# arancormonk/dsd-neo

Measured on AMD Instinct MI355X. Metric: I/Q Msamples/s end-to-end (demod->FEC->MBE) per GPU; % HBM roofline, higher is better.
Workload: dtype f32

## Files before the change

### dsd-neo_amd/csrc/ddn_rx.hip

```cpp

#include <hip/hip_runtime.h>
#include <cstdio>
#include <cstdlib>
#include <mutex>
#include <stdint.h>

#include "ddn_device.h"
#include "ddn_p25h_dev.h"
#include "ddn_slicer_dev.h"
#include "ddn_tables_p25.h"

using ddn_sl::two_max_insert;
using ddn_sl::two_min_insert;

#define DDN_RXW_RAW (1 << 30)
namespace {
constexpr int TS = 64;
constexpr int SS = 128;
constexpr int MS = 1024;
constexpr int NT = DDN_P25_FILTER_TAPS;
constexpr int QCAP = 10;
constexpr uint32_t kSyncBits = 0xFB30A0u;

__constant__ uint32_t c_taps[NT];
// ... 573 lines not shown
v_max2(float a, float b) {
    float r;
    asm("v_max_f32 %0, %1, %2" : "=v"(r) : "v"(a), "v"(b));
    return r;
}
__device__ __forceinline__ float
v_min3(float a, float b, float c) {
    float r;
    asm("v_min3_f32 %0, %1, %2, %3" : "=v"(r) : "v"(a), "v"(b), "v"(c));
    return r;
}
__device__ __forceinline__ float
v_max3(float a, float b, float c) {
    float r;
    asm("v_max3_f32 %0, %1, %2, %3" : "=v"(r) : "v"(a), "v"(b), "v"(c));
    return r;
}
__device__ __forceinline__ float
v_med3(float a, float b, float c) {
    float r;
    asm("v_med3_f32 %0, %1, %2, %3" : "=v"(r) : "v"(a), "v"(b), "v"(c));
    return r;
}
__device__ __forceinline__ void
helper_idle(float& spin, bool sleep_instead, int sleep_arg) {
    if (sleep_instead) {
        if (sleep_arg >= 4) {
            __builtin_amdgcn_s_sleep(4);
        } else {
            __builtin_amdgcn_s_sleep(1);
        }
        return;
    }
#pragma unroll
    for (int k = 0; k < 12; k++) {
        asm volatile("v_max_f32 %0, %0, %0" : "+v"(spin));
    }
}
__device__ __forceinline__ float
div5_exact(float x) {
    const float y = 0.2f;
    const float q = x * y;
    const float r = __builtin_fmaf(-5.0f, q, x);
    return __builtin_fmaf(r, y, q);
}


#ifndef DDN_RX_CYCLES
#define DDN_RX_CYCLES 0
#endif

template <int CPW, bool SMALL = false>
struct LdsW {
    static constexpr int TW = CPW <= 8 ? 128 : 64, RTW = 3 * TW;
    static constexpr int WMW = TW == 128 ? (SMALL ? 40 : 64) : (SMALL ? 24 : 32);
    static constexpr int QTW = TW == 128 ? 40 : 20;
    float sb[SS][CPW];
    float lb[24][CPW];
    float sh[24][CPW];
    float raw[CPW][RTW + TW + 13];
    float flt[CPW][RTW + TW + 13];
    alignas(16) float q[2][QTW][CPW][4];
    int qn[2][4];
    int qo[2][CPW];
    alignas(16) float sfx[2][WMW][CPW][4];
    int sidx0[2][CPW];
};

template <int CPW>
struct LdsH {
    float hh[ddn_p25h::HN][CPW][3];
    int req_seq[CPW], req_kind[CPW], req_hw[CPW], req_n[CPW], req_o[CPW], req_neg[CPW], req_nc[CPW];
    int rsp_seq[CPW], rsp_ext[CPW], rsp_more[CPW];
#if DDN_RX_CYCLES
    int req_t[CPW], rsp_t[CPW], rsp_pick[CPW];
#endif
    int tile_done[4];
    int hwid[8];
    int ready[4];
    int fready[4];
    int staged[4];
    float hh_dummy[CPW][4];
    ddn_p25h::Scratch sc;
};

template <int CPW, bool HM, int NRW_T = (HM ? 2 : 1)>
__global__ __launch_bounds__(HM ? 64 * (NRW_T + 2) * (NRW_T == 4 ? 2 : 1) : 192) __attribute__((amdgpu_waves_per_eu(NRW_T == 4 ? 3 : 2))) void
k_p25_rxw(const float* __restrict__ raw, const float* __restrict__ filt, const float* __restrict__ prev_tail,
          float* __restrict__ fstale, long n,
          size_t stride, int n_channels, DdnRxConfig cfg, DdnRxState* __restrict__ state, float* __restrict__ sbuf_store,
          float* __restrict__ lbuf_store, float* __restrict__ shist_store, float* __restrict__ minring,
          float* __restrict__ maxring, uint8_t* __restrict__ rec, uint8_t* __restrict__ flags,
          int32_t* __restrict__ counts, size_t max_sym, const int32_t* __restrict__ lock_cfg,
          DdnP25HState* __restrict__ hstate, float* __restrict__ hh_store, int32_t* __restrict__ events,
          int32_t* __restrict__ n_events) {
    using LW = LdsW<CPW, HM>;
    constexpr int TW = LW::TW, RTW = LW::RTW, WMW = LW::WMW, QTW = LW::QTW;
    (void)RTW;
    extern __shared__ unsigned char smem_all[];
    constexpr int LTHREADS = HM ? 64 * (NRW_T + 2) : 192;
    constexpr size_t LBYTES = HM ? ((((sizeof(LW) + 15) & ~(size_t)15) + sizeof(LdsH<CPW>) + 15) & ~(size_t)15) : sizeof(LW);
    const int lhalf = (NRW_T == 4) ? (int)(threadIdx.x / LTHREADS) : 0;
    const int ltid = (int)threadIdx.x - lhalf * LTHREADS;
    const int lblock = (NRW_T == 4) ? (int)blockIdx.x * 2 + lhalf : (int)blockIdx.x;
    unsigned char* smem_raw = smem_all + (size_t)lhalf * LBYTES;
    LW& L = *reinterpret_cast<LW*>(smem_raw);
    LdsH<CPW>& H = *reinterpret_cast<LdsH<CPW>*>(smem_raw + ((sizeof(LW) + 15) & ~(size_t)15));
    const int lane = ltid & 63;
    const bool fuse_mf = HM && LdsW<CPW, HM>::TW == 128 && cfg.use_filter != 0 && filt == nullptr;
    int wave_role = ltid >> 6;
    if (HM && !(cfg.dbg & 524288)) {
        unsigned hwid;
        asm volatile("s_getreg_b32 %0, hwreg(HW_REG_HW_ID)" : "=s"(hwid));
        if (lane == 0) {
            H.hwid[ltid >> 6] = (int)hwid;
        }
        __syncthreads();
        int seen = 0, slot_of_simd0 = 0;
        for (int w = 0; w < 4; w++) {
            const int v = H.hwid[w];
            seen |= 1 << ((v >> 4) & 3);
            if (((v >> 4) & 3) == 0) {
                slot_of_simd0 = v & 15;
            }
        }
        if (NRW_T == 2 && seen == 15) {
            wave_role = ((int)((hwid >> 4) & 3) - 2 * (slot_of_simd0 & 1)) & 3;
        }
        if (NRW_T == 4) {
            constexpr int NW = NRW_T + 2;
            const int me = ltid >> 6, my_simd = (int)((hwid >> 4) & 3);
            int cnt[4] = {0, 0, 0, 0}, my_rank = 0;
            for (int w = 0; w < NW; w++) {
                const int sd = (H.hwid[w] >> 4) & 3;
                cnt[sd]++;
                my_rank += (w < me && sd == my_simd) ? 1 : 0;
            }
            const bool good = cnt[0] >= 1 && cnt[1] >= 1 && cnt[2] >= 1 && cnt[3] >= 1 && cnt[0] <= 2 && cnt[1] <= 2 && cnt[2] <= 2 && cnt[3] <= 2;
            if (good) {
                int before = 0;
                for (int sd = 0; sd < my_simd; sd++) {
                    before += my_rank == 0 ? 1 : (cnt[sd] == 2 ? 1 : 0);
                }
                wave_role = my_rank == 0 ? before : NRW_T + before;
            }
        }
    }
    const bool hwave = HM && wave_role == NRW_T + 1;
    if (HM && hwave) {
        const int ch0 = lblock * CPW;
        const int ch = ch0 + lane;
        auto wg_barrier = [&]() {
            __builtin_amdgcn_fence(__ATOMIC_RELEASE, "workgroup");
            __builtin_amdgcn_s_barrier();
            __builtin_amdgcn_fence(__ATOMIC_ACQUIRE, "workgroup");
        };
        __builtin_amdgcn_s_setprio(3);
    DdnP25HState hs = DdnP25HState{};
    int h_served = 0, h_nev = 0;
    const bool hlive = hwave && lane < CPW && ch < n_channels;
    {
        if (hlive) {
            hs = hstate[ch];
        }
        for (int k = lane; k < ddn_p25h::HN * CPW * 3; k += 64) {
            const int w = k % 3, c = (k / 3) % CPW, slot = k / (3 * CPW);
            H.hh[slot][c][w] = (ch0 + c < n_channels) ? hh_store[((size_t)(ch0 + c) * ddn_p25h::HN + slot) * 3 + w] : 0.0f;
        }
        if (lane < CPW) {
            H.req_seq[lane] = 0;
            H.rsp_seq[lane] = 0;
        }
        ddn_p25h::crc_cols_fill(H.sc.crc_cols, lane);
        if (lane == 0) {
            for (int w = 0; w < 4; w++) {
                H.tile_done[w] = DDN_RXW_RAW;
                H.ready[w] = 1;
                H.fready[w] = 0;
                H.staged[w] = 1;
            }
            ddn_nid::gf_fill(H.sc.ex, H.sc.lg);
            ddn_nid::chase_masks_fill(H.sc.masks);
        }
    }
        wg_barrier();
        wg_barrier();
    int dbg_pend = 0, dbg_free = 0;
    auto serve = [&](int c, int seq) {
        using namespace ddn_p25h;
        Scratch& sc = H.sc;
        const int kind = H.req_kind[c], hw = H.req_hw[c], nsym = H.req_n[c], o_dec = H.req_o[c], neg = H.req_neg[c];
        const int gch = ch0 + c;
        const long long dbg_t0 = (cfg.dbg & 65536) ? (long long)clock64() : 0;
#if DDN_RX_CYCLES
        if (lane == c) {
            const int since_req = (int)dbg_t0 - H.req_t[c];
            const int since_free = dbg_free == 0 ? 0x7fffffff : (int)((unsigned)(int)dbg_t0 - (unsigned)dbg_free);
            H.rsp_pick[c] = (cfg.dbg & 268435456) ? 1000 * dbg_pend : ((cfg.dbg & 536870912) ? (since_req < since_free ? since_req : since_free) : since_req);
        }
#endif
        int dbg_path = 0;
        long long dbg_s[3] = {0, 0, 0};
        auto dbg_stamp = [&](int k) {
            if (cfg.dbg & 131072) {
                dbg_s[k] = (long long)clock64() - dbg_t0;
            }
        };
        int phase = __shfl(hs.phase, c), block = __shfl(hs.block, c), end = __shfl(hs.end, c), sk0 = __shfl(hs.skipdibit, c);
        int nac = __shfl(hs.nac, c), p2cc = __shfl(hs.p2_cc, c);
        int nev = __shfl(h_nev, c);
        if (H.req_nc[c]) {
            nac = 0;
        }
        if (kind == 1) {
            phase = PH_NID;
        }
        int ext = 0, more = 0;
        int ev_kind = 0, ev_a = 0, ev_b = 0;
        int32_t pay0 = 0, pay1 = 0, pay2 = 0, pay3 = 0;
        auto slice_at = [&](int i, int& d, int& relb, int& l0, int& l1) {
            int slot = hw - nsym + i;
            slot += slot < 0 ? HN : 0;
            const float* e = &H.hh[slot][c][0];
            const float mx = e[1], mn = e[2];
            const float center = (mx + mn) / 2.0f;
            const ddn_sl::Thr th = {center, ((mx - center) * 5.0f / 8.0f) + center, ((mn - center) * 5.0f / 8.0f) + center, mx, mn};
            ddn_sl::slice_soft(e[0], th, neg, d, relb, l0, l1);
        };
        if (phase == PH_NID) {
            bool nid_done = false;
            ddn_nid::NidRes r = {0, 0, 0, 0};
            {
                int hd = 0;
                if (lane < 33 && lane != 11) {
                    int slot = hw - nsym + lane;
                    slot += slot < 0 ? HN : 0;
                    const float* e = &H.hh[slot][c][0];
                    const float mx = e[1], mn = e[2], x = e[0];
                    const float center = (mx + mn) / 2.0f;
                    const float umid = ((mx - center) * 5.0f / 8.0f) + center, lmid = ((mn - center) * 5.0f / 8.0f) + center;
                    hd = (x > center) ? ((x > umid) ? (neg ? 3 : 1) : (neg ? 2 : 0)) : ((x < lmid) ? (neg ? 1 : 3) : (neg ? 0 : 2));
                }
                const unsigned long long bh = __ballot(hd & 2), bl = __ballot(hd & 1);
                const uint32_t ph = (uint32_t)((bh & 0x7FFull) | ((bh >> 12) << 11)), pl = (uint32_t)((bl & 0x7FFull) | ((bl >> 12) << 11));
                auto spread = [](uint32_t v) {
                    uint64_t x = v;
                    x = (x | (x << 16)) & 0x0000FFFF0000FFFFull;
                    x = (x | (x << 8)) & 0x00FF00FF00FF00FFull;
                    x = (x | (x << 4)) & 0x0F0F0F0F0F0F0F0Full;
                    x = (x | (x << 2)) & 0x3333333333333333ull;
                    x = (x | (x << 1)) & 0x5555555555555555ull;
                    return x;
                };
                const uint64_t both = spread(ph) | (spread(pl) << 1);
                const uint64_t w0 = both & 0x7FFFFFFFFFFFFFFFull;
                const int par0 = (int)(both >> 63);
                dbg_stamp(0);
                if (ddn_nid::bch_63_16_is_codeword(w0)) {
                    r = ddn_nid::nid_fields(w0, 0, par0);
                    nid_done = r.status > 0;
                }
                dbg_stamp(2);
// ... 93 lines not shown
                ev_a = block;
                ev_b = crc_ok | (((by[0] >> 8) & 0xFF) << 8) | (((last << 8) | sel) << 16);
                block++;
                if (last || block >= 3) {
                    phase = PH_IDLE;
                } else {
                    ext = 101;
                    more = 1;
                }
            } else {
                if (crc_ok) {
                    const int sap = (by[0] >> 8) & 0x3F, blks = (by[1] >> 16) & 0x7F;
                    end = blks + 1;
                    if ((sap == 61 || sap == 63) && blks > 10) {
                        end = 4;
                    }
                }
                ev_kind = EV_MPDU;
                ev_a = crc_ok;
                ev_b = (end & 0xFFFF) | (byte0 << 16);
                block = 1;
                int total = 0;
                for (int bi = 1; bi < end; bi++) {
                    int ska;
                    total += mpdu_block_symbols(sk0, ska);
                    sk0 = ska;
                }
                ext = total;
                more = 0;
                phase = PH_IDLE;
            }
        } else {
            phase = PH_IDLE;
        }
        if (lane == c) {
            hs.phase = phase;
            hs.block = block;
            hs.end = end;
            hs.skipdibit = sk0;
            hs.nac = nac;
            hs.p2_cc = p2cc;
            h_served = seq;
            H.rsp_ext[c] = ext;
            H.rsp_more[c] = more;
#if DDN_RX_CYCLES
            H.rsp_t[c] = (int)clock64();
#endif
        }
#if DDN_RX_CYCLES
        dbg_free = (int)clock64();
#endif
        if (lane == c) {
            __builtin_amdgcn_fence(__ATOMIC_RELEASE, "workgroup", "local");
            __hip_atomic_store(&H.rsp_seq[c], seq, __ATOMIC_RELAXED, __HIP_MEMORY_SCOPE_WORKGROUP);
            if (ev_kind) {
                if (nev < cfg.max_events && gch < n_channels) {
                    int32_t* e = events + ((size_t)gch * cfg.max_events + nev) * 4;
                    e[0] = o_dec;
                    e[1] = ev_kind;
                    e[2] = ev_a;
                    e[3] = ev_b;
                    if (cfg.event_data) {
                        *reinterpret_cast<int4*>(cfg.event_data + ((size_t)gch * cfg.max_events + nev) * 4) = make_int4(pay0, pay1, pay2, pay3);
                    }
                    if (cfg.dbg & 65536) {
                        e[2] = dbg_path;
                        e[3] = (int)((long long)clock64() - dbg_t0);
                        if (cfg.dbg & 131072) {
                            e[2] = dbg_path | ((int)(dbg_s[0] >> 4) << 4);
                            e[3] = (int)(dbg_s[1] >> 4) | ((int)(dbg_s[2] >> 4) << 16);
                        }
#if DDN_RX_CYCLES
                        if (cfg.dbg & 1073741824) {
                            e[2] = H.rsp_pick[c];
                        }
#endif
                    }
                }
                h_nev = nev + 1;
            }
        }
    };

        constexpr int LPR_H = CPW / NRW_T;
        constexpr int NPASS = LPR_H / 2;
        static_assert(LPR_H % 2 == 0, "the filter pass takes the channels of a recurrence wave in pairs");
        typedef float mf2h __attribute__((ext_vector_type(2)));
        auto mf_pass = [&](int h, int t, int p) {
            const int slot = t % 3;
            const int cA = h * LPR_H + 2 * p, cB = cA + 1;
            const float* ra = &L.raw[cA][TW + slot * TW + 2 * lane - (NT - 1)];
            const float* rb = &L.raw[cB][TW + slot * TW + 2 * lane - (NT - 1)];
            mf2h accA = {0.0f, 0.0f}, accB = {0.0f, 0.0f};
            {
                constexpr int G = 7;
                static_assert(NT == 13 * G, "thirteen groups of seven taps");
                uint32_t la = (uint32_t)(uintptr_t)(const __attribute__((address_space(3))) float*)ra;
                uint32_t lb = (uint32_t)(uintptr_t)(const __attribute__((address_space(3))) float*)rb;
#define DDN_MF_LOAD(d, e, a, b)                                                                                                    \
    asm volatile("ds_read2_b32 %0, %14 offset1:1\n\tds_read2_b32 %7, %15 offset1:1\n\t"                                          \
                 "ds_read2_b32 %1, %14 offset0:1 offset1:2\n\tds_read2_b32 %8, %15 offset0:1 offset1:2\n\t"                     \
                 "ds_read2_b32 %2, %14 offset0:2 offset1:3\n\tds_read2_b32 %9, %15 offset0:2 offset1:3\n\t"                     \
                 "ds_read2_b32 %3, %14 offset0:3 offset1:4\n\tds_read2_b32 %10, %15 offset0:3 offset1:4\n\t"                    \
                 "ds_read2_b32 %4, %14 offset0:4 offset1:5\n\tds_read2_b32 %11, %15 offset0:4 offset1:5\n\t"                    \
                 "ds_read2_b32 %5, %14 offset0:5 offset1:6\n\tds_read2_b32 %12, %15 offset0:5 offset1:6\n\t"                    \
                 "ds_read2_b32 %6, %14 offset0:6 offset1:7\n\tds_read2_b32 %13, %15 offset0:6 offset1:7"                        \
                 : "=&v"(d[0]), "=&v"(d[1]), "=&v"(d[2]), "=&v"(d[3]), "=&v"(d[4]), "=&v"(d[5]), "=&v"(d[6]), "=&v"(e[0]),         \
                   "=&v"(e[1]), "=&v"(e[2]), "=&v"(e[3]), "=&v"(e[4]), "=&v"(e[5]), "=&v"(e[6])                                    \
                 : "v"(a), "v"(b)                                                                                                  \
                 : "memory")
#define DDN_MF_WAIT(d, e, cnt)                                                                                                     \
    asm volatile("s_waitcnt lgkmcnt(" cnt ")"                                                                                      \
                 : "+v"(d[0]), "+v"(d[1]), "+v"(d[2]), "+v"(d[3]), "+v"(d[4]), "+v"(d[5]), "+v"(d[6]), "+v"(e[0]), "+v"(e[1]),     \
                   "+v"(e[2]), "+v"(e[3]), "+v"(e[4]), "+v"(e[5]), "+v"(e[6]))
                mf2h xa0[G], xb0[G], xa1[G], xb1[G];
                DDN_MF_LOAD(xa0, xb0, la, lb);
#pragma unroll
                for (int g = 0; g < 13; g++) {
                    mf2h* ca = (g & 1) ? xa1 : xa0;
                    mf2h* cb = (g & 1) ? xb1 : xb0;
                    if (g + 1 < 13) {
                        la += 4u * G;
                        lb += 4u * G;
                        if (g & 1) {
                            DDN_MF_LOAD(xa0, xb0, la, lb);
                        } else {
                            DDN_MF_LOAD(xa1, xb1, la, lb);
                        }
                        DDN_MF_WAIT(ca, cb, "14");
                    } else {
                        DDN_MF_WAIT(ca, cb, "0");
                    }
#pragma unroll
                    for (int k = 0; k < G; k++) {
                        const float tp = __uint_as_float(ddn_p25_filter_bits[g * G + k]);
                        const mf2h tt = {tp, tp};
                        const mf2h pa = tt * ca[k], pb = tt * cb[k];
                        accA += pa;
                        accB += pb;
                    }
                }
#undef DDN_MF_LOAD
#undef DDN_MF_WAIT
            }
            float* fa = &L.flt[cA][TW + slot * TW + 2 * lane];
            float* fb = &L.flt[cB][TW + slot * TW + 2 * lane];
            fa[0] = accA.x;
            fa[1] = accA.y;
            fb[0] = accB.x;
            fb[1] = accB.y;
            if (slot == 2) {
                fa[-3 * TW] = accA.x;
                fa[1 - 3 * TW] = accA.y;
                fb[-3 * TW] = accB.x;
                fb[1 - 3 * TW] = accB.y;
            }
        };
        const int n_tiles = (int)((n + TW - 1) / TW);
        int mfj[NRW_T], mfp[NRW_T];
        for (int w = 0; w < NRW_T; w++) {
            mfj[w] = 0;
            mfp[w] = 0;
        }
        float idle_spin = 0.0f;
#if DDN_RX_CYCLES
        long long dbg_mf[8] = {0, 0, 0, 0, 0, 0, 0, 0};
#endif
        while (true) {
            const int rq = (lane < CPW) ? __hip_atomic_load(&H.req_seq[lane], __ATOMIC_RELAXED, __HIP_MEMORY_SCOPE_WORKGROUP) : 0;
            const unsigned long long pend = __ballot(lane < CPW && rq != h_served);
            if (pend != 0) {
                __builtin_amdgcn_fence(__ATOMIC_ACQUIRE, "workgroup");
                const int c = __ffsll((long long)pend) - 1;
                dbg_pend = __popcll(pend);
#if DDN_RX_CYCLES
                const long long sv_t0 = (long long)clock64();
#endif
                serve(c, __shfl(rq, c));
#if DDN_RX_CYCLES
                dbg_mf[2] += (long long)clock64() - sv_t0;
                dbg_mf[3]++;
#endif
                continue;
            }
            bool did = false;
            if (fuse_mf) {
                int hsel = -1, jsel = 0x7fffffff;
#pragma unroll
                for (int h = 0; h < NRW_T; h++) {
                    if (mfj[h] < n_tiles && mfj[h] < jsel
                        && __hip_atomic_load(&H.staged[h], __ATOMIC_RELAXED, __HIP_MEMORY_SCOPE_WORKGROUP) > mfj[h]) {
                        hsel = h;
                        jsel = mfj[h];
                    }
                }
                if (hsel >= 0) {
                    __builtin_amdgcn_fence(__ATOMIC_ACQUIRE, "workgroup");
                    int pj = 0;
#pragma unroll
                    for (int h = 0; h < NRW_T; h++) {
                        pj = h == hsel ? mfp[h] : pj;
                    }
#if DDN_RX_CYCLES
                    const long long mf_t0 = (long long)clock64();
#endif
                    mf_pass(hsel, jsel, pj);
#if DDN_RX_CYCLES
                    dbg_mf[0] += (long long)clock64() - mf_t0;
                    dbg_mf[1]++;
#endif
                    pj++;
                    const bool tile_filtered = pj == NPASS;
#pragma unroll
                    for (int h = 0; h < NRW_T; h++) {
                        if (h == hsel) {
                            mfp[h] = tile_filtered ? 0 : pj;
                            mfj[h] += tile_filtered ? 1 : 0;
                        }
                    }
                    if (tile_filtered) {
                        __builtin_amdgcn_fence(__ATOMIC_RELEASE, "workgroup");
                        if (lane == 0) {
                            __hip_atomic_store(&H.fready[hsel], jsel + 1, __ATOMIC_RELAXED, __HIP_MEMORY_SCOPE_WORKGROUP);
                        }
                    }
                    did = true;
                }
            }
            if (did) {
                continue;
            }
            bool all_done = true;
            for (int w = 0; w < NRW_T; w++) {
                all_done = all_done
                           && (__hip_atomic_load(&H.tile_done[w], __ATOMIC_ACQUIRE, __HIP_MEMORY_SCOPE_WORKGROUP) & (DDN_RXW_RAW - 1)) >= n_tiles;
            }
            if (all_done) {
                break;
            }
            helper_idle(idle_spin, (cfg.dbg & 8388608) != 0, 4);
#if DDN_RX_CYCLES
            dbg_mf[4]++;
#endif
        }
#if DDN_RX_CYCLES
        if ((cfg.dbg & 8192) && lane == 0) {
            uint8_t* d = rec + ((size_t)ch0 + 1) * max_sym * 10 - 448;
            for (int k = 0; k < 64; k++) {
                d[k] = reinterpret_cast<const uint8_t*>(dbg_mf)[k];
            }
        }
#endif
    {
        if (hlive) {
            hstate[ch] = hs;
            n_events[ch] = h_nev;
        }
        for (int k = lane; k < ddn_p25h::HN * CPW * 3; k += 64) {
            const int w = k % 3, c = (k / 3) % CPW, slot = k / (3 * CPW);
            if (ch0 + c < n_channels) {
                hh_store[((size_t)(ch0 + c) * ddn_p25h::HN + slot) * 3 + w] = H.hh[slot][c][w];
            }
        }
    }
        return;
    }
    constexpr int NRW = NRW_T;
    constexpr int LPR = CPW / NRW;
    const int wave = wave_role;
    const bool loader = wave == NRW;
    const bool winprep = wave == (HM ? NRW : NRW + 1);
    const bool recur = wave < NRW;
    const int rw = recur ? wave : 0;
    const int ch0 = lblock * CPW;
    const int ln = rw * LPR + (lane < LPR ? lane : 0);
    const int ch = ch0 + ln;
    const bool live = recur && lane < LPR && ch < n_channels;
    const bool use_flt = cfg.use_filter != 0;
    const bool ld_flt = use_flt && filt != nullptr;
    const bool raw_always = !ld_flt || (cfg.dbg & 16384) != 0;
    const float inf = __builtin_inff();
    if (recur && !(cfg.dbg & 32768)) {
        __builtin_amdgcn_s_setprio(3);
    }

    DdnRxState s;
    if (live) {
        s = state[ch];
        for (int k = 0; k < SS; k++) {
            L.sb[k][ln] = sbuf_store[(size_t)k * n_channels + ch];
        }
        for (int k = 0; k < 24; k++) {
            L.lb[k][ln] = lbuf_store[(size_t)k * n_channels + ch];
            L.sh[k][ln] = shist_store[(size_t)k * n_channels + ch];
        }
    } else {
        s = DdnRxState{};
    }
    float wabs = 0.0f;
    if (live) {
        L.sidx0[0][ln] = s.sidx;
        for (int k = 0; k < SS; k++) {
            wabs = fmaxf(wabs, fabsf(L.sb[k][ln]));
        }
    }
    auto stage = [&](long t0, int slot) {
        const int tn = (int)((n - t0) < TW ? (n - t0) : TW);
        constexpr int RPP = CPW < 16 ? CPW : 16;
#pragma unroll
        for (int half = 0; half < TW / 64; half++) {
// ... 621 lines not shown
        int job[NRW];
        for (int h = 0; h < NRW; h++) {
            job[h] = 0;
        }
        float idle_spin = 0.0f;
        auto jobs_left = [&]() {
            bool any = false;
            for (int h = 0; h < NRW; h++) {
                any = any || job[h] <= n_tiles;
            }
            return any;
        };
        while (jobs_left()) {
            bool served = false;
#pragma unroll
            for (int h = 0; h < NRW; h++) {
                const int j = job[h];
                const int tdw = __hip_atomic_load(&H.tile_done[h], __ATOMIC_RELAXED, __HIP_MEMORY_SCOPE_WORKGROUP);
                if (j > n_tiles || (tdw & (DDN_RXW_RAW - 1)) < j) {
                    continue;
                }
                __builtin_amdgcn_fence(__ATOMIC_ACQUIRE, "workgroup");
                const long long w0 = (DDN_RX_CYCLES && (cfg.dbg & 8192)) ? (long long)clock64() : 0;
                if (j < n_tiles) {
                    long long c0 = w0;
                    StageRegs sg;
                    if (j + 1 < n_tiles) {
                        stage_half_load((long)(j + 1) * TW, h, sg, (tdw & DDN_RXW_RAW) != 0);
                    }
                    if (DDN_RX_CYCLES && (cfg.dbg & 8192)) {
                        const long long c1 = (long long)clock64();
                        dbg_cyc[0] += c1 - c0;
                        c0 = c1;
                    }
                    if (offload && j > 0 && !(cfg.dbg & 512)) {
                        drain_half((j - 1) & 1, h);
                    }
                    if (DDN_RX_CYCLES && (cfg.dbg & 8192)) {
                        const long long c1 = (long long)clock64();
                        dbg_cyc[1] += c1 - c0;
                        c0 = c1;
                    }
                    if (fuse_mf) {
                        if (j + 1 < n_tiles) {
                            stage_half_store(j + 1, h, sg);
                        }
                        __builtin_amdgcn_fence(__ATOMIC_RELEASE, "workgroup");
                        if (lane == 0) {
                            __hip_atomic_store(&H.staged[h], j + 2, __ATOMIC_RELAXED, __HIP_MEMORY_SCOPE_WORKGROUP);
                        }
                        if (DDN_RX_CYCLES && (cfg.dbg & 8192)) {
                            const long long c1 = (long long)clock64();
                            dbg_cyc[0] += c1 - c0;
                            c0 = c1;
                        }
                    }
                    if (j >= 1 && !(cfg.dbg & 256)) {
                        compute_sfx_half(j & 1, j & 1, h);
                    }
                    if (DDN_RX_CYCLES && (cfg.dbg & 8192)) {
                        const long long c1 = (long long)clock64();
                        dbg_cyc[2] += c1 - c0;
                        c0 = c1;
                    }
                    if (!fuse_mf && j + 1 < n_tiles) {
                        stage_half_store(j + 1, h, sg);
                    }
                    if (DDN_RX_CYCLES && (cfg.dbg & 8192)) {
                        dbg_cyc[0] += (long long)clock64() - c0;
                    }
                    __builtin_amdgcn_fence(__ATOMIC_RELEASE, "workgroup");
                    if (lane == 0) {
                        __hip_atomic_store(&H.ready[h], j + 2, __ATOMIC_RELAXED, __HIP_MEMORY_SCOPE_WORKGROUP);
                    }
                } else if (offload && n_tiles > 0) {
                    drain_half((n_tiles - 1) & 1, h);
                }
                if (DDN_RX_CYCLES && (cfg.dbg & 8192)) {
                    dbg_busy += (long long)clock64() - w0;
                }
                job[h] = j + 1;
                served = true;
            }
            if (!served) {
                const long long w0 = (DDN_RX_CYCLES && (cfg.dbg & 8192)) ? (long long)clock64() : 0;
                helper_idle(idle_spin, (cfg.dbg & 8388608) != 0, 1);
                if (DDN_RX_CYCLES && (cfg.dbg & 8192)) {
                    dbg_wait += (long long)clock64() - w0;
                }
            }
        }
        it = n_tiles;
    } else
    for (t0 = 0; t0 < n; t0 += TW, it++) {
        const long long dbg_t0 = (DDN_RX_CYCLES && (cfg.dbg & 8192)) ? (long long)clock64() : 0;
        const int tn = (int)((n - t0) < TW ? (n - t0) : TW);
        const bool more = (t0 + TW) < n;
        long long dbg_spin = 0;
        if (HM) {
            const long long w0 = (DDN_RX_CYCLES && (cfg.dbg & 8192)) ? (long long)clock64() : 0;
            while (__hip_atomic_load(&H.ready[rw], __ATOMIC_RELAXED, __HIP_MEMORY_SCOPE_WORKGROUP) <= it
                   || (fuse_mf && __hip_atomic_load(&H.fready[rw], __ATOMIC_RELAXED, __HIP_MEMORY_SCOPE_WORKGROUP) <= it)) {
                __builtin_amdgcn_s_sleep(1);
            }
            __builtin_amdgcn_fence(__ATOMIC_ACQUIRE, "workgroup");
            if (DDN_RX_CYCLES && (cfg.dbg & 8192)) {
                dbg_spin = (long long)clock64() - w0;
            }
        }
        if (loader || winprep) {
            if (loader) {
                if (more) {
                    stage(t0 + TW, (it + 1) % 3);
                }
                if (offload && it > 0 && !(cfg.dbg & 512)) {
                    drain((it - 1) & 1);
                }
            }
            if (winprep) {
                if (it >= 1 && !(cfg.dbg & 256)) {
                    compute_sfx(it & 1, it & 1);
                }
            }
        } else {
            const int base = TW + (it % 3) * TW;
            auto rd = [&](const float* row, int j) { return row[base + j]; };
            auto cold_limit = [&]() {
                if (!s.filter_on) {
                    return -2147483647;
                }
                const long long d = (long long)(NT - 1) - (abs0 + t0 - s.filt_start);
                return d <= -2147483647LL ? -2147483647 : (d > 1000000LL ? 1000000 : (int)d);
            };
            cold_until = cold_limit();
            if (it >= 1) {
                pp1 = pc1, pp2 = pc2, pp3 = pc3, pp4 = pc4;
                npp = npc;
                sbuf_sel = (it - 1) & 1;
            }
            pc1 = inf, pc2 = inf, pc3 = -inf, pc4 = -inf;
            npc = 0;
            tk = 0;
            itq = it & 1;
            o_tile = o;
            if (live && offload) {
                L.qo[it & 1][ln] = o;
            }
            int guard = 0;
            bool gblocked = false;
            bool respin = false;
            int blk_o = -1;
            while (true) {
                const long long dbg_p0 = (DDN_RX_CYCLES && (cfg.dbg & 8192)) ? (long long)clock64() : 0;
                long long dbg_p1 = 0;
                if (HM && __any(hwait)) {
                    if (hwait
                        && __hip_atomic_load(&H.rsp_seq[ln], __ATOMIC_RELAXED, __HIP_MEMORY_SCOPE_WORKGROUP) == hseq) {
                        __builtin_amdgcn_fence(__ATOMIC_ACQUIRE, "workgroup", "local");
                        const int ext = H.rsp_ext[ln];
                        hwait = false;
                        if ((cfg.dbg & 65536) && !(cfg.dbg & (67108864 | 134217728))) {
                            s.dbg_wait += (long long)clock64();
                        }
#if DDN_RX_CYCLES
                        if (cfg.dbg & 67108864) {
                            s.dbg_wait += (long long)((int)clock64() - H.rsp_t[ln]);
                        }
                        if (cfg.dbg & 134217728) {
                            s.dbg_wait += (long long)H.rsp_pick[ln];
                        }
#endif
                        if (ext > 0) {
                            s.lock_left = ext;
                            s.hn = ext;
                            s.hphase = H.rsp_more[ln] ? 2 : 0;
                        } else {
                            s.hphase = 0;
                            frame_end();
                        }
                    }
                    if (__any(hwait) && (LPR > 4) != ((cfg.dbg & 262144) != 0)) {
                        __builtin_amdgcn_s_sleep(1);
                        continue;
                    }
                }
// ... 992 lines not shown
                    s.in_symbol = 0;
                    commit_pre(sym);
                    int fl = 0;
                    float q_max = 0.0f, q_min = 0.0f;
                    if (s.have_sync) {
                        commit_inframe(sym, done_snap, fl, q_max, q_min);
                    } else {
                        commit_hunt(sym, done_snap, fl);
                    }
                    emit(sym, fl, q_max, q_min);
                }
                gblocked = gblocked || blocked;
            }
            if ((DDN_RX_CYCLES && (cfg.dbg & 8192)) && dbg_kind >= 0) {
                dbg_cyc[dbg_kind] += (long long)clock64() - dbg_prev;
                dbg_n[dbg_kind]++;
                dbg_kind = -1;
            }
            if (offload && lane == 0) {
                L.qn[it & 1][rw] = (tk - 1) < QTW ? (tk - 1) : QTW;
            }
            if (live) {
                L.sidx0[(it + 1) & 1][ln] = s.sidx;
                sp -= TW;
            }
            if (HM) {
                const bool want = live
                                  && (!s.filter_on || cold_until > 0 || (!s.have_sync && s.hunt_pos + 64 >= 1800) || raw_always);
                const int raw_bit = __any(want) ? DDN_RXW_RAW : 0;
                __builtin_amdgcn_fence(__ATOMIC_RELEASE, "workgroup");
                if (lane == 0) {
                    __hip_atomic_store(&H.tile_done[rw], (it + 1) | raw_bit, __ATOMIC_RELAXED, __HIP_MEMORY_SCOPE_WORKGROUP);
                }
            }
        }
        if (DDN_RX_CYCLES && (cfg.dbg & 8192)) {
            const long long t1 = (long long)clock64();
            if (!HM) {
                __syncthreads();
            }
            dbg_busy += t1 - dbg_t0 - dbg_spin;
            dbg_wait += (long long)clock64() - t1 + dbg_spin;
        } else if (!HM) {
            __syncthreads();
        }
    }
    if ((DDN_RX_CYCLES && (cfg.dbg & 8192)) && lane == 0) {
        uint8_t* d = rec + ((size_t)ch0 + 1) * max_sym * 10 - 192 + (wave < NRW ? (wave ? 1 : 0) : 2) * 64;
        const long long v[8] = {dbg_busy, dbg_wait, dbg_cyc[0], dbg_cyc[1], dbg_cyc[2], dbg_n[0], dbg_n[1], dbg_n[2]};
        for (int k = 0; k < 64; k++) {
            d[k] = reinterpret_cast<const uint8_t*>(v)[k];
        }
        if (wave == 0) {
            uint8_t* d2 = rec + ((size_t)ch0 + 1) * max_sym * 10 - 256;
            for (int k = 0; k < 64; k++) {
                d2[k] = reinterpret_cast<const uint8_t*>(dbg_sec)[k];
                d2[k - 64] = reinterpret_cast<const uint8_t*>(dbg_run)[k];
                d2[k - 128] = reinterpret_cast<const uint8_t*>(dbg_blk)[k];
                d2[k - 256] = reinterpret_cast<const uint8_t*>(dbg_ent)[k];
            }
        }
    }
    if (!HM && loader && offload && it > 0) {
        drain((it - 1) & 1);
    }
    if (live) {
        if (s.have_sync) {
            s.umid = ((s.max - s.center) * 5.0f / 8.0f) + s.center;
            s.lmid = ((s.min - s.center) * 5.0f / 8.0f) + s.center;
        }
        s.n_abs = abs0 + n;
        state[ch] = s;
        counts[ch] = o;
        for (int k = 0; k < SS; k++) {
            sbuf_store[(size_t)k * n_channels + ch] = L.sb[k][ln];
        }
        for (int k = 0; k < 24; k++) {
            lbuf_store[(size_t)k * n_channels + ch] = L.lb[k][ln];
            shist_store[(size_t)k * n_channels + ch] = L.sh[k][ln];
        }
    }
}

template <int CPW, bool HM, int NRW_T = (HM ? 2 : 1)>
static hipError_t
launch_rxw(const float* raw, const float* filt, const float* prev_tail, float* fstale, long n, size_t stride, int n_channels,
           const DdnRxConfig& cfg, DdnRxState* state, float* sbuf_store, float* lbuf_store, float* shist_store,
           float* minring, float* maxring, uint8_t* rec, uint8_t* flags, int32_t* counts, size_t max_sym, const int32_t* lock_cfg,
           DdnP25HState* hstate, float* hh_store, int32_t* events, int32_t* n_events, hipStream_t st) {
    const size_t shm1 = HM ? (((((sizeof(LdsW<CPW, true>) + 15) & ~(size_t)15) + sizeof(LdsH<CPW>)) + 15) & ~(size_t)15) : sizeof(LdsW<CPW>);
    const size_t shm = shm1 * (NRW_T == 4 ? 2 : 1);
    const unsigned lblocks = (unsigned)((n_channels + CPW - 1) / CPW);
    const unsigned nblocks = NRW_T == 4 ? (lblocks + 1) / 2 : lblocks;
    const unsigned nthreads = HM ? 64 * (NRW_T + 2) * (NRW_T == 4 ? 2 : 1) : 192;
    if (HM && (cfg.sym_rate <= 0 || cfg.out_rate / cfg.sym_rate < 9)) {
        return hipErrorInvalidValue;
    }
    hipError_t e = hipFuncSetAttribute(reinterpret_cast<const void*>(&k_p25_rxw<CPW, HM, NRW_T>),
                                       hipFuncAttributeMaxDynamicSharedMemorySize, (int)shm);
    if (e != hipSuccess) {
        return e;
    }
    if (DDN_EXP_ENV("DDN_RX_OCC")) {
        int nb = -1;
        hipFuncAttributes fa;
        (void)hipOccupancyMaxActiveBlocksPerMultiprocessor(&nb, reinterpret_cast<const void*>(&k_p25_rxw<CPW, HM, NRW_T>), (int)nthreads, shm);
        (void)hipFuncGetAttributes(&fa, reinterpret_cast<const void*>(&k_p25_rxw<CPW, HM, NRW_T>));
        fprintf(stderr, "k_p25_rxw<%d,%d,%d>: %d blocks per CU, %d regs, %zu B dynamic LDS, %zu B static\n", CPW, (int)HM, NRW_T, nb, fa.numRegs, shm, fa.sharedSizeBytes);
    }
    hipLaunchKernelGGL((k_p25_rxw<CPW, HM, NRW_T>), dim3(nblocks), dim3(nthreads), shm, st, raw,
                       filt, prev_tail, fstale, n, stride, n_channels, cfg, state, sbuf_store, lbuf_store, shist_store, minring,
                       maxring, rec, flags, counts, max_sym, lock_cfg, hstate, hh_store, events, n_events);
    return hipGetLastError();
}

template <int CPW>
static hipError_t
launch_rx(const float* raw, const float* filt, const float* prev_tail, float* fstale, long n, size_t stride, int n_channels,
          const DdnRxConfig& cfg, DdnRxState* state, float* sbuf_store, float* lbuf_store, float* shist_store,
          float* minring, float* maxring, uint8_t* rec, uint8_t* flags, int32_t* counts, size_t max_sym, const int32_t* lock_cfg,
          hipStream_t st) {
    const size_t shm = sizeof(Lds<CPW>);
    hipError_t e = hipFuncSetAttribute(reinterpret_cast<const void*>(&k_p25_rx<CPW>),
                                       hipFuncAttributeMaxDynamicSharedMemorySize, (int)shm);
    if (e != hipSuccess) {
        return e;
    }
    hipLaunchKernelGGL(k_p25_rx<CPW>, dim3((unsigned)((n_channels + CPW - 1) / CPW)), dim3(128), shm, st, raw, filt,
                       prev_tail, fstale, n, stride, n_channels, cfg, state, sbuf_store, lbuf_store, shist_store, minring,
                       maxring, rec, flags, counts, max_sym, lock_cfg);
    return hipGetLastError();
}

static inline bool
use_filter_row_missing(const DdnRxConfig* cfg, const float* filt) {
    return cfg->use_filter && !filt;
}

static int
handler_mode_cpw(int channels_per_wave, int n_channels) {
    int cpw = channels_per_wave;
    if (const char* e = DDN_EXP_ENV("DDN_RX_CPW")) {
        cpw = atoi(e);
    }
    if (cpw != 4 && cpw != 8 && cpw != 16) {
        cpw = n_channels <= 4 * 512 ? 4 : 8;
    }
    return cpw;
}

extern "C" int
ddn_dev_p25_rx_fuses_filter(const DdnRxConfig* cfg, int channels_per_wave, int n_channels) {
    return cfg && cfg->handlers && cfg->use_filter && handler_mode_cpw(channels_per_wave, n_channels) <= 8
               ? 1
               : 0;
}

extern "C" hipError_t
ddn_dev_p25_rx(const float* raw, const float* filt, const float* prev_tail, float* fstale, long n, size_t stride, int n_channels,
               const DdnRxConfig* cfg, DdnRxState* state, float* sbuf_store, float* lbuf_store, float* shist_store,
               float* minring, float* maxring, uint8_t* rec, uint8_t* flags, int32_t* counts, size_t max_sym,
               int channels_per_wave, const int32_t* lock_cfg, DdnP25HState* hstate, float* hh_store, int32_t* events,
               int32_t* n_events, hipStream_t st) {
    if (n_channels <= 0 || n <= 0) {
        return hipSuccess;
    }
    if ((unsigned long long)n_channels * (unsigned long long)MS * 4ull > 0xFFFFFFFFull) {
        return hipErrorInvalidValue;
    }
    {
        static std::mutex mu;
        static bool taps_up[64] = {};
        int dev = 0;
        hipError_t e = hipGetDevice(&dev);
        if (e != hipSuccess) {
            return e;
        }
        std::lock_guard<std::mutex> lock(mu);
        if (dev < 0 || dev >= 64 || !taps_up[dev]) {
            e = hipMemcpyToSymbol(HIP_SYMBOL(c_taps), ddn_p25_filter_bits, sizeof(uint32_t) * NT);
            if (e != hipSuccess) {
                return e;
            }
            if (dev >= 0 && dev < 64) {
                taps_up[dev] = true;
            }
        }
    }
    int cpw = channels_per_wave;
    if (const char* e = DDN_EXP_ENV("DDN_RX_CPW")) {
        cpw = atoi(e);
    }
    const int whole = cfg->sym_rate > 0 ? cfg->out_rate / cfg->sym_rate : 0;
// ... 70 lines not shown
```

Baseline: 25570.

## Share fused matched-filter passes between handler and stager waves via atomic work queue

The fused matched-filter work moves out of per-wave private counters into a shared LDS queue. Both the handler wave and idle stager waves claim filter passes with compare-and-swap and mark completion per pass. A new FUSE template parameter makes the fused path a compile-time instantiation, so non-fused kernels drop the dead code. The aim is to spread the filter load over idle waves so recurrence waves wait less, at the cost of atomic contention and a noinline call in the stager loop.

```diff
diff --git a/dsd-neo_amd/csrc/ddn_rx.hip b/dsd-neo_amd/csrc/ddn_rx.hip
--- a/dsd-neo_amd/csrc/ddn_rx.hip
+++ b/dsd-neo_amd/csrc/ddn_rx.hip
@@ -679,9 +679,134 @@
     int staged[4];
     float hh_dummy[CPW][4];
     ddn_p25h::Scratch sc;
+    int mf_next[4];
+    int mf_done[4][8];
 };
 
-template <int CPW, bool HM, int NRW_T = (HM ? 2 : 1)>
+typedef float mf2h __attribute__((ext_vector_type(2)));
+template <int CPW, int NRW_T>
+__device__ __forceinline__ void
+rxw_mf_pass(LdsW<CPW, true>& L, int lane, int h, int t, int p) {
+    constexpr int TW = LdsW<CPW, true>::TW;
+    constexpr int LPR_H = CPW / NRW_T;
+    static_assert(LPR_H % 2 == 0, "the filter pass takes the channels of a recurrence wave in pairs");
+    const int slot = t % 3;
+    const int cA = h * LPR_H + 2 * p, cB = cA + 1;
+    const float* ra = &L.raw[cA][TW + slot * TW + 2 * lane - (NT - 1)];
+    const float* rb = &L.raw[cB][TW + slot * TW + 2 * lane - (NT - 1)];
+    mf2h accA = {0.0f, 0.0f}, accB = {0.0f, 0.0f};
+    {
+        constexpr int G = 7;
+        static_assert(NT == 13 * G, "thirteen groups of seven taps");
+        uint32_t la = (uint32_t)(uintptr_t)(const __attribute__((address_space(3))) float*)ra;
+        uint32_t lb = (uint32_t)(uintptr_t)(const __attribute__((address_space(3))) float*)rb;
+#define DDN_MF_LOAD(d, e, a, b)                                                                                                    \
+    asm volatile("ds_read2_b32 %0, %14 offset1:1\n\tds_read2_b32 %7, %15 offset1:1\n\t"                                          \
+                 "ds_read2_b32 %1, %14 offset0:1 offset1:2\n\tds_read2_b32 %8, %15 offset0:1 offset1:2\n\t"                     \
+                 "ds_read2_b32 %2, %14 offset0:2 offset1:3\n\tds_read2_b32 %9, %15 offset0:2 offset1:3\n\t"                     \
+                 "ds_read2_b32 %3, %14 offset0:3 offset1:4\n\tds_read2_b32 %10, %15 offset0:3 offset1:4\n\t"                    \
+                 "ds_read2_b32 %4, %14 offset0:4 offset1:5\n\tds_read2_b32 %11, %15 offset0:4 offset1:5\n\t"                    \
+                 "ds_read2_b32 %5, %14 offset0:5 offset1:6\n\tds_read2_b32 %12, %15 offset0:5 offset1:6\n\t"                    \
+                 "ds_read2_b32 %6, %14 offset0:6 offset1:7\n\tds_read2_b32 %13, %15 offset0:6 offset1:7"                        \
+                 : "=&v"(d[0]), "=&v"(d[1]), "=&v"(d[2]), "=&v"(d[3]), "=&v"(d[4]), "=&v"(d[5]), "=&v"(d[6]), "=&v"(e[0]),         \
+                   "=&v"(e[1]), "=&v"(e[2]), "=&v"(e[3]), "=&v"(e[4]), "=&v"(e[5]), "=&v"(e[6])                                    \
+                 : "v"(a), "v"(b)                                                                                                  \
+                 : "memory")
+#define DDN_MF_WAIT(d, e, cnt)                                                                                                     \
+    asm volatile("s_waitcnt lgkmcnt(" cnt ")"                                                                                      \
+                 : "+v"(d[0]), "+v"(d[1]), "+v"(d[2]), "+v"(d[3]), "+v"(d[4]), "+v"(d[5]), "+v"(d[6]), "+v"(e[0]), "+v"(e[1]),     \
+                   "+v"(e[2]), "+v"(e[3]), "+v"(e[4]), "+v"(e[5]), "+v"(e[6]))
+        mf2h xa0[G], xb0[G], xa1[G], xb1[G];
+        DDN_MF_LOAD(xa0, xb0, la, lb);
+#pragma unroll
+        for (int g = 0; g < 13; g++) {
+            mf2h* ca = (g & 1) ? xa1 : xa0;
+            mf2h* cb = (g & 1) ? xb1 : xb0;
+            if (g + 1 < 13) {
+                la += 4u * G;
+                lb += 4u * G;
+                if (g & 1) {
+                    DDN_MF_LOAD(xa0, xb0, la, lb);
+                } else {
+                    DDN_MF_LOAD(xa1, xb1, la, lb);
+                }
+                DDN_MF_WAIT(ca, cb, "14");
+            } else {
+                DDN_MF_WAIT(ca, cb, "0");
+            }
+#pragma unroll
+            for (int k = 0; k < G; k++) {
+                const float tp = __uint_as_float(ddn_p25_filter_bits[g * G + k]);
+                const mf2h tt = {tp, tp};
+                const mf2h pa = tt * ca[k], pb = tt * cb[k];
+                accA += pa;
+                accB += pb;
+            }
+        }
+#undef DDN_MF_LOAD
+#undef DDN_MF_WAIT
+    }
+    float* fa = &L.flt[cA][TW + slot * TW + 2 * lane];
+    float* fb = &L.flt[cB][TW + slot * TW + 2 * lane];
+    fa[0] = accA.x;
+    fa[1] = accA.y;
+    fb[0] = accB.x;
+    fb[1] = accB.y;
+    if (slot == 2) {
+        fa[-3 * TW] = accA.x;
+        fa[1 - 3 * TW] = accA.y;
+        fb[-3 * TW] = accB.x;
+        fb[1 - 3 * TW] = accB.y;
+    }
+}
+
+template <int CPW, int NRW_T>
+__device__ __forceinline__ int
+rxw_mf_take(LdsW<CPW, true>& L, LdsH<CPW>& H, int lane, int mf_tiles) {
+    constexpr int NPASS = CPW / NRW_T / 2;
+    static_assert(LdsW<CPW, true>::TW != 128 || 4 * NPASS <= 8, "H.mf_done holds four tiles' pass words");
+    int hsel = -1, jsel = 0x7fffffff, vsel = 0;
+#pragma unroll
+    for (int h = 0; h < NRW_T; h++) {
+        const int v = __builtin_amdgcn_readfirstlane(__hip_atomic_load(&H.mf_next[h], __ATOMIC_RELAXED, __HIP_MEMORY_SCOPE_WORKGROUP));
+        const int j = v / NPASS;
+        if (j < mf_tiles && j < jsel
+            && __builtin_amdgcn_readfirstlane(__hip_atomic_load(&H.staged[h], __ATOMIC_RELAXED, __HIP_MEMORY_SCOPE_WORKGROUP)) > j) {
+            hsel = h;
+            jsel = j;
+            vsel = v;
+        }
+    }
+    if (hsel < 0) {
+        return 0;
+    }
+    int won = 0;
+    if (lane == 0) {
+        int expect = vsel;
+        won = __hip_atomic_compare_exchange_strong(&H.mf_next[hsel], &expect, vsel + 1, __ATOMIC_RELAXED, __ATOMIC_RELAXED,
+                                                   __HIP_MEMORY_SCOPE_WORKGROUP)
+                  ? 1
+                  : 0;
+    }
+    if (!__builtin_amdgcn_readfirstlane(won)) {
+        return 1;
+    }
+    __builtin_amdgcn_fence(__ATOMIC_ACQUIRE, "workgroup");
+    const int pj = vsel % NPASS;
+    rxw_mf_pass<CPW, NRW_T>(L, lane, hsel, jsel, pj);
+    __builtin_amdgcn_fence(__ATOMIC_RELEASE, "workgroup");
+    if (lane == 0) {
+        __hip_atomic_store(&H.mf_done[hsel][(jsel & 3) * NPASS + pj], jsel + 1, __ATOMIC_RELAXED, __HIP_MEMORY_SCOPE_WORKGROUP);
+    }
+    return 2;
+}
+template <int CPW, int NRW_T>
+__device__ __noinline__ int
+rxw_mf_take_call(LdsW<CPW, true>& L, LdsH<CPW>& H, int lane, int mf_tiles) {
+    return rxw_mf_take<CPW, NRW_T>(L, H, lane, mf_tiles);
+}
+
+template <int CPW, bool HM, int NRW_T = (HM ? 2 : 1), bool FUSE = false>
 __global__ __launch_bounds__(HM ? 64 * (NRW_T + 2) * (NRW_T == 4 ? 2 : 1) : 192) __attribute__((amdgpu_waves_per_eu(NRW_T == 4 ? 3 : 2))) void
 k_p25_rxw(const float* __restrict__ raw, const float* __restrict__ filt, const float* __restrict__ prev_tail,
           float* __restrict__ fstale, long n,
@@ -704,7 +829,34 @@
     LW& L = *reinterpret_cast<LW*>(smem_raw);
     LdsH<CPW>& H = *reinterpret_cast<LdsH<CPW>*>(smem_raw + ((sizeof(LW) + 15) & ~(size_t)15));
     const int lane = ltid & 63;
-    const bool fuse_mf = HM && LdsW<CPW, HM>::TW == 128 && cfg.use_filter != 0 && filt == nullptr;
+    static_assert(!FUSE || (HM && LdsW<CPW, HM>::TW == 128), "the filter in the loop: handler mode, 128-sample tiles");
+    constexpr bool fuse_mf = FUSE;
+    constexpr int NPASS = CPW / NRW_T / 2;
+    const int mf_tiles = (int)((n + TW - 1) / TW);
+    const bool mf_by_handler = fuse_mf && ((cfg.dbg & 1) || !(cfg.dbg & 2));
+    const bool mf_by_stager = fuse_mf && !(cfg.dbg & 1);
+    auto mf_take = [&]() -> int {
+        if constexpr (FUSE) {
+            return rxw_mf_take<CPW, NRW_T>(L, H, lane, mf_tiles);
+        } else {
+            return 0;
+        }
+    };
+    auto mf_take_call = [&]() -> int {
+        if constexpr (FUSE) {
+            return rxw_mf_take_call<CPW, NRW_T>(L, H, lane, mf_tiles);
+        } else {
+            return 0;
+        }
+    };
+    auto mf_tile_done = [&](int h, int t) {
+        bool all = true;
+#pragma unroll
+        for (int p = 0; p < NPASS; p++) {
+            all = all && __hip_atomic_load(&H.mf_done[h][(t & 3) * NPASS + p], __ATOMIC_RELAXED, __HIP_MEMORY_SCOPE_WORKGROUP) > t;
+        }
+        return all;
+    };
     int wave_role = ltid >> 6;
     if (HM && !(cfg.dbg & 524288)) {
         unsigned hwid;
@@ -773,8 +925,11 @@
             for (int w = 0; w < 4; w++) {
                 H.tile_done[w] = DDN_RXW_RAW;
                 H.ready[w] = 1;
-                H.fready[w] = 0;
                 H.staged[w] = 1;
+                H.mf_next[w] = 0;
+                for (int k = 0; k < 8; k++) {
+                    H.mf_done[w][k] = 0;
+                }
             }
             ddn_nid::gf_fill(H.sc.ex, H.sc.lg);
             ddn_nid::chase_masks_fill(H.sc.masks);
@@ -1034,86 +1189,7 @@
         }
     };
 
-        constexpr int LPR_H = CPW / NRW_T;
-        constexpr int NPASS = LPR_H / 2;
-        static_assert(LPR_H % 2 == 0, "the filter pass takes the channels of a recurrence wave in pairs");
-        typedef float mf2h __attribute__((ext_vector_type(2)));
-        auto mf_pass = [&](int h, int t, int p) {
-            const int slot = t % 3;
-            const int cA = h * LPR_H + 2 * p, cB = cA + 1;
-            const float* ra = &L.raw[cA][TW + slot * TW + 2 * lane - (NT - 1)];
-            const float* rb = &L.raw[cB][TW + slot * TW + 2 * lane - (NT - 1)];
-            mf2h accA = {0.0f, 0.0f}, accB = {0.0f, 0.0f};
-            {
-                constexpr int G = 7;
-                static_assert(NT == 13 * G, "thirteen groups of seven taps");
-                uint32_t la = (uint32_t)(uintptr_t)(const __attribute__((address_space(3))) float*)ra;
-                uint32_t lb = (uint32_t)(uintptr_t)(const __attribute__((address_space(3))) float*)rb;
-#define DDN_MF_LOAD(d, e, a, b)                                                                                                    \
-    asm volatile("ds_read2_b32 %0, %14 offset1:1\n\tds_read2_b32 %7, %15 offset1:1\n\t"                                          \
-                 "ds_read2_b32 %1, %14 offset0:1 offset1:2\n\tds_read2_b32 %8, %15 offset0:1 offset1:2\n\t"                     \
-                 "ds_read2_b32 %2, %14 offset0:2 offset1:3\n\tds_read2_b32 %9, %15 offset0:2 offset1:3\n\t"                     \
-                 "ds_read2_b32 %3, %14 offset0:3 offset1:4\n\tds_read2_b32 %10, %15 offset0:3 offset1:4\n\t"                    \
-                 "ds_read2_b32 %4, %14 offset0:4 offset1:5\n\tds_read2_b32 %11, %15 offset0:4 offset1:5\n\t"                    \
-                 "ds_read2_b32 %5, %14 offset0:5 offset1:6\n\tds_read2_b32 %12, %15 offset0:5 offset1:6\n\t"                    \
-                 "ds_read2_b32 %6, %14 offset0:6 offset1:7\n\tds_read2_b32 %13, %15 offset0:6 offset1:7"                        \
-                 : "=&v"(d[0]), "=&v"(d[1]), "=&v"(d[2]), "=&v"(d[3]), "=&v"(d[4]), "=&v"(d[5]), "=&v"(d[6]), "=&v"(e[0]),         \
-                   "=&v"(e[1]), "=&v"(e[2]), "=&v"(e[3]), "=&v"(e[4]), "=&v"(e[5]), "=&v"(e[6])                                    \
-                 : "v"(a), "v"(b)                                                                                                  \
-                 : "memory")
-#define DDN_MF_WAIT(d, e, cnt)                                                                                                     \
-    asm volatile("s_waitcnt lgkmcnt(" cnt ")"                                                                                      \
-                 : "+v"(d[0]), "+v"(d[1]), "+v"(d[2]), "+v"(d[3]), "+v"(d[4]), "+v"(d[5]), "+v"(d[6]), "+v"(e[0]), "+v"(e[1]),     \
-                   "+v"(e[2]), "+v"(e[3]), "+v"(e[4]), "+v"(e[5]), "+v"(e[6]))
-                mf2h xa0[G], xb0[G], xa1[G], xb1[G];
-                DDN_MF_LOAD(xa0, xb0, la, lb);
-#pragma unroll
-                for (int g = 0; g < 13; g++) {
-                    mf2h* ca = (g & 1) ? xa1 : xa0;
-                    mf2h* cb = (g & 1) ? xb1 : xb0;
-                    if (g + 1 < 13) {
-                        la += 4u * G;
-                        lb += 4u * G;
-                        if (g & 1) {
-                            DDN_MF_LOAD(xa0, xb0, la, lb);
-                        } else {
-                            DDN_MF_LOAD(xa1, xb1, la, lb);
-                        }
-                        DDN_MF_WAIT(ca, cb, "14");
-                    } else {
-                        DDN_MF_WAIT(ca, cb, "0");
-                    }
-#pragma unroll
-                    for (int k = 0; k < G; k++) {
-                        const float tp = __uint_as_float(ddn_p25_filter_bits[g * G + k]);
-                        const mf2h tt = {tp, tp};
-                        const mf2h pa = tt * ca[k], pb = tt * cb[k];
-                        accA += pa;
-                        accB += pb;
-                    }
-                }
-#undef DDN_MF_LOAD
-#undef DDN_MF_WAIT
-            }
-            float* fa = &L.flt[cA][TW + slot * TW + 2 * lane];
-            float* fb = &L.flt[cB][TW + slot * TW + 2 * lane];
-            fa[0] = accA.x;
-            fa[1] = accA.y;
-            fb[0] = accB.x;
-            fb[1] = accB.y;
-            if (slot == 2) {
-                fa[-3 * TW] = accA.x;
-                fa[1 - 3 * TW] = accA.y;
-                fb[-3 * TW] = accB.x;
-                fb[1 - 3 * TW] = accB.y;
-            }
-        };
-        const int n_tiles = (int)((n + TW - 1) / TW);
-        int mfj[NRW_T], mfp[NRW_T];
-        for (int w = 0; w < NRW_T; w++) {
-            mfj[w] = 0;
-            mfp[w] = 0;
-        }
+        const int n_tiles = mf_tiles;
         float idle_spin = 0.0f;
 #if DDN_RX_CYCLES
         long long dbg_mf[8] = {0, 0, 0, 0, 0, 0, 0, 0};
@@ -1136,48 +1212,18 @@
                 continue;
             }
             bool did = false;
-            if (fuse_mf) {
-                int hsel = -1, jsel = 0x7fffffff;
-#pragma unroll
-                for (int h = 0; h < NRW_T; h++) {
-                    if (mfj[h] < n_tiles && mfj[h] < jsel
-                        && __hip_atomic_load(&H.staged[h], __ATOMIC_RELAXED, __HIP_MEMORY_SCOPE_WORKGROUP) > mfj[h]) {
-                        hsel = h;
-                        jsel = mfj[h];
-                    }
-                }
-                if (hsel >= 0) {
-                    __builtin_amdgcn_fence(__ATOMIC_ACQUIRE, "workgroup");
-                    int pj = 0;
-#pragma unroll
-                    for (int h = 0; h < NRW_T; h++) {
-                        pj = h == hsel ? mfp[h] : pj;
-                    }
+            if (mf_by_handler) {
 #if DDN_RX_CYCLES
-                    const long long mf_t0 = (long long)clock64();
+                const long long mf_t0 = (long long)clock64();
 #endif
-                    mf_pass(hsel, jsel, pj);
+                const int took = mf_take();
 #if DDN_RX_CYCLES
+                if (took == 2) {
                     dbg_mf[0] += (long long)clock64() - mf_t0;
                     dbg_mf[1]++;
+                }
 #endif
-                    pj++;
-                    const bool tile_filtered = pj == NPASS;
-#pragma unroll
-                    for (int h = 0; h < NRW_T; h++) {
-                        if (h == hsel) {
-                            mfp[h] = tile_filtered ? 0 : pj;
-                            mfj[h] += tile_filtered ? 1 : 0;
-                        }
-                    }
-                    if (tile_filtered) {
-                        __builtin_amdgcn_fence(__ATOMIC_RELEASE, "workgroup");
-                        if (lane == 0) {
-                            __hip_atomic_store(&H.fready[hsel], jsel + 1, __ATOMIC_RELAXED, __HIP_MEMORY_SCOPE_WORKGROUP);
-                        }
-                    }
-                    did = true;
-                }
+                did = took != 0;
             }
             if (did) {
                 continue;
@@ -1965,6 +2011,17 @@
                 job[h] = j + 1;
                 served = true;
             }
+            if (!served && mf_by_stager) {
+                const long long w0 = (DDN_RX_CYCLES && (cfg.dbg & 8192)) ? (long long)clock64() : 0;
+                const int took = mf_take_call();
+                if (DDN_RX_CYCLES && (cfg.dbg & 8192) && took == 2) {
+                    const int dt = (int)((long long)clock64() - w0);
+                    dbg_busy += dt;
+                    dbg_n[0]++;
+                    dbg_n[1] += dt;
+                }
+                served = took != 0;
+            }
             if (!served) {
                 const long long w0 = (DDN_RX_CYCLES && (cfg.dbg & 8192)) ? (long long)clock64() : 0;
                 helper_idle(idle_spin, (cfg.dbg & 8388608) != 0, 1);
@@ -1983,7 +2040,7 @@
         if (HM) {
             const long long w0 = (DDN_RX_CYCLES && (cfg.dbg & 8192)) ? (long long)clock64() : 0;
             while (__hip_atomic_load(&H.ready[rw], __ATOMIC_RELAXED, __HIP_MEMORY_SCOPE_WORKGROUP) <= it
-                   || (fuse_mf && __hip_atomic_load(&H.fready[rw], __ATOMIC_RELAXED, __HIP_MEMORY_SCOPE_WORKGROUP) <= it)) {
+                   || (fuse_mf && !mf_tile_done(rw, it))) {
                 __builtin_amdgcn_s_sleep(1);
             }
             __builtin_amdgcn_fence(__ATOMIC_ACQUIRE, "workgroup");
@@ -3142,12 +3199,19 @@
     }
 }
 
-template <int CPW, bool HM, int NRW_T = (HM ? 2 : 1)>
+template <int CPW, bool HM, int NRW_T = (HM ? 2 : 1), bool FUSE = false>
 static hipError_t
 launch_rxw(const float* raw, const float* filt, const float* prev_tail, float* fstale, long n, size_t stride, int n_channels,
            const DdnRxConfig& cfg, DdnRxState* state, float* sbuf_store, float* lbuf_store, float* shist_store,
            float* minring, float* maxring, uint8_t* rec, uint8_t* flags, int32_t* counts, size_t max_sym, const int32_t* lock_cfg,
            DdnP25HState* hstate, float* hh_store, int32_t* events, int32_t* n_events, hipStream_t st) {
+    if constexpr (HM && !FUSE && LdsW<CPW, HM>::TW == 128) {
+        if (cfg.use_filter != 0 && filt == nullptr) {
+            return launch_rxw<CPW, HM, NRW_T, true>(raw, filt, prev_tail, fstale, n, stride, n_channels, cfg, state, sbuf_store, lbuf_store,
+                                                    shist_store, minring, maxring, rec, flags, counts, max_sym, lock_cfg, hstate,
+                                                    hh_store, events, n_events, st);
+        }
+    }
     const size_t shm1 = HM ? (((((sizeof(LdsW<CPW, true>) + 15) & ~(size_t)15) + sizeof(LdsH<CPW>)) + 15) & ~(size_t)15) : sizeof(LdsW<CPW>);
     const size_t shm = shm1 * (NRW_T == 4 ? 2 : 1);
     const unsigned lblocks = (unsigned)((n_channels + CPW - 1) / CPW);
@@ -3156,7 +3220,7 @@
     if (HM && (cfg.sym_rate <= 0 || cfg.out_rate / cfg.sym_rate < 9)) {
         return hipErrorInvalidValue;
     }
-    hipError_t e = hipFuncSetAttribute(reinterpret_cast<const void*>(&k_p25_rxw<CPW, HM, NRW_T>),
+    hipError_t e = hipFuncSetAttribute(reinterpret_cast<const void*>(&k_p25_rxw<CPW, HM, NRW_T, FUSE>),
                                        hipFuncAttributeMaxDynamicSharedMemorySize, (int)shm);
     if (e != hipSuccess) {
         return e;
@@ -3164,11 +3228,11 @@
     if (DDN_EXP_ENV("DDN_RX_OCC")) {
         int nb = -1;
         hipFuncAttributes fa;
-        (void)hipOccupancyMaxActiveBlocksPerMultiprocessor(&nb, reinterpret_cast<const void*>(&k_p25_rxw<CPW, HM, NRW_T>), (int)nthreads, shm);
-        (void)hipFuncGetAttributes(&fa, reinterpret_cast<const void*>(&k_p25_rxw<CPW, HM, NRW_T>));
+        (void)hipOccupancyMaxActiveBlocksPerMultiprocessor(&nb, reinterpret_cast<const void*>(&k_p25_rxw<CPW, HM, NRW_T, FUSE>), (int)nthreads, shm);
+        (void)hipFuncGetAttributes(&fa, reinterpret_cast<const void*>(&k_p25_rxw<CPW, HM, NRW_T, FUSE>));
         fprintf(stderr, "k_p25_rxw<%d,%d,%d>: %d blocks per CU, %d regs, %zu B dynamic LDS, %zu B static\n", CPW, (int)HM, NRW_T, nb, fa.numRegs, shm, fa.sharedSizeBytes);
     }
-    hipLaunchKernelGGL((k_p25_rxw<CPW, HM, NRW_T>), dim3(nblocks), dim3(nthreads), shm, st, raw,
+    hipLaunchKernelGGL((k_p25_rxw<CPW, HM, NRW_T, FUSE>), dim3(nblocks), dim3(nthreads), shm, st, raw,
                        filt, prev_tail, fstale, n, stride, n_channels, cfg, state, sbuf_store, lbuf_store, shist_store, minring,
                        maxring, rec, flags, counts, max_sym, lock_cfg, hstate, hh_store, events, n_events);
     return hipGetLastError();
```

Result: no change. 25670 (median of 6 runs) (+0.4%).
